# achraf-15/neural_image_compression

Hardware: AMD Instinct MI355X
Metric: images/sec (256x256 RGB, batch 32) fwd+bwd (higher is better)
Workload: dtype f32; 1 GPU; cfg2: JointAutoregressiveHierarchical(M=192,K=1) fwd+rd_loss(lambda=0.01)+bwd+Adam, 32x3x256x256 per GPU, fp32; global_batch=32, parallelism=dp1, step=eager (autograd)

## Files before the change

neural_image_compression_amd/csrc/lic_gdn.hip:

```cpp
#include "lic_common.h"

namespace {

constexpr int GD_BM = 64;
constexpr int GD_BK = 16;

struct GdnParams {
  const float* x;
  const float* g;
  const float* norm;
  const float* w;
  const float* beta;
  const float* res;
  float* out;
  float* out2;
  float* cs_t;
  float* cs_dx;
  long P;
  int inverse;
};

template <int TN, int MODE>
__global__ __launch_bounds__(256) void gdn_kernel(const GdnParams p) {
  static_assert(MODE == 0, "forward only");
  constexpr int C = 64 * TN;
  constexpr int LDX = C + 4;
  constexpr int NCH = C / GD_BK;
  constexpr int SLOTS = GD_BM * C / 4 / 256;
  __shared__ __attribute__((aligned(16))) float smem[GD_BM * LDX];
  const int tid = threadIdx.x, lane = tid & 63;
  const int wave = __builtin_amdgcn_readfirstlane(tid >> 6);
  const int wm0 = (wave >> 1) * 32, wn0 = (wave & 1) * (32 * TN);
  const int li = lane & 31, lh = lane >> 5;
  const long m0 = (long)blockIdx.x * GD_BM;
  const bool inv = p.inverse != 0;

  {
    f32x4 a[SLOTS];
#pragma unroll
    for (int u = 0; u < SLOTS; ++u) {
      const int idx = u * 256 + tid;
      const int row = idx / (C / 4), c4 = (idx - row * (C / 4)) * 4;
      const bool ok = m0 + row < p.P;
      a[u] = *reinterpret_cast<const f32x4*>(p.x + (ok ? (m0 + row) * C + c4 : 0L));
      if (!ok) a[u] = f32x4{0.f, 0.f, 0.f, 0.f};
    }
#pragma unroll
    for (int u = 0; u < SLOTS; ++u) {
      const int idx = u * 256 + tid;
      const int row = idx / (C / 4), c4 = (idx - row * (C / 4)) * 4;
      *reinterpret_cast<f32x4*>(&smem[row * LDX + c4]) = a[u];
    }
  }
  __syncthreads();

  f32x16 acc[TN];
#pragma unroll
  for (int b = 0; b < TN; ++b)
#pragma unroll
    for (int r = 0; r < 16; ++r) acc[b][r] = 0.0f;
  const float* glane = p.w + ((long)(wn0 >> 5) * 512 + lane * 4);
  const float* xrow = smem + (wm0 + li) * LDX + lh * 8;
  f32x4 g0[TN][2], g1[TN][2];
  auto load_g = [&](f32x4 (&rg)[TN][2], int c) {
    const float* src = glane + (long)(c < NCH ? c : NCH - 1) * C * GD_BK;
#pragma unroll
    for (int b = 0; b < TN; ++b) {
      rg[b][0] = *reinterpret_cast<const f32x4*>(src + b * 512);
      rg[b][1] = *reinterpret_cast<const f32x4*>(src + b * 512 + 256);
    }
  };
  auto pool = [&](int c, const f32x4 (&rg)[TN][2]) {
    f32x4 a0 = *reinterpret_cast<const f32x4*>(xrow + c * GD_BK);
    f32x4 a1 = *reinterpret_cast<const f32x4*>(xrow + c * GD_BK + 4);
    a0 = a0 * a0;
    a1 = a1 * a1;
#pragma unroll
    for (int t = 0; t < 8; ++t)
#pragma unroll
      for (int b = 0; b < TN; ++b)
        acc[b] = __builtin_amdgcn_mfma_f32_32x32x2f32((t < 4 ? a0 : a1)[t & 3], rg[b][t >> 2][t & 3], acc[b], 0, 0, 0);
  };
  load_g(g0, 0);
#pragma unroll 1
  for (int c = 0; c < NCH; c += 2) {
    load_g(g1, c + 1);
    pool(c, g0);
    load_g(g0, c + 2);
    pool(c + 1, g1);
  }

  __shared__ __attribute__((aligned(16))) float patch[4][1024];
  float* stg = patch[wave];
  const int c4 = (lane & 7) * 4, r8 = lane >> 3;
  f32x4 csum[TN];
#pragma unroll
  for (int b = 0; b < TN; ++b) csum[b] = f32x4{0.f, 0.f, 0.f, 0.f};
#pragma unroll
  for (int b = 0; b < TN; ++b) {
#pragma unroll
    for (int r = 0; r < 16; ++r) stg[((r & 3) + 8 * (r >> 2) + 4 * lh) * 32 + li] = acc[b][r];
    __builtin_amdgcn_wave_barrier();
    const int col = wn0 + b * 32 + c4;
#pragma unroll
    for (int it = 0; it < 4; ++it) {
      const int rr = it * 8 + r8;
      const long pix = m0 + wm0 + rr;
      if (pix >= p.P) continue;
      const f32x4 s4 = *reinterpret_cast<const f32x4*>(&stg[rr * 32 + c4]);
      const long off = pix * C + col;
      const f32x4 n4 = s4 + *reinterpret_cast<const f32x4*>(p.beta + col);
      const f32x4 x4 = *reinterpret_cast<const f32x4*>(&smem[(wm0 + rr) * LDX + col]);
      f32x4 o;
#pragma unroll
      for (int e = 0; e < 4; ++e)
        o[e] = x4[e] * (inv ? __builtin_amdgcn_sqrtf(n4[e]) : __builtin_amdgcn_rsqf(n4[e]));
      if (p.out2) *reinterpret_cast<f32x4*>(p.out2 + off) = n4;
      if (p.res) o += *reinterpret_cast<const f32x4*>(p.res + off);
      *reinterpret_cast<f32x4*>(p.out + off) = o;
    }
    __builtin_amdgcn_wave_barrier();
  }
}

template <int TN>
__global__ __launch_bounds__(256, 2) void gdn_bwd_reg_kernel(const GdnParams p) {
  constexpr int C = 64 * TN;
  constexpr int LDX = C + 4;
  constexpr int NCH = C / GD_BK;
  __shared__ __attribute__((aligned(16))) float smem[GD_BM * LDX];
  const int tid = threadIdx.x, lane = tid & 63;
  const int wave = __builtin_amdgcn_readfirstlane(tid >> 6);
  const int wm0 = (wave >> 1) * 32, wn0 = (wave & 1) * (32 * TN);
  const int li = lane & 31, lh = lane >> 5;
  const int c4 = (lane & 7) * 4, r8 = lane >> 3;
  const long m0 = (long)blockIdx.x * GD_BM;
  const bool inv = p.inverse != 0;

  f32x4 u[TN][4], xx[TN][4];
#pragma unroll
  for (int b = 0; b < TN; ++b) {
    f32x4 gg[4], nn[4];
    bool ok[4];
#pragma unroll
    for (int it = 0; it < 4; ++it) {
      const long pix = m0 + wm0 + it * 8 + r8;
      ok[it] = pix < p.P;
      const long off = ok[it] ? pix * C + wn0 + b * 32 + c4 : 0L;
      xx[b][it] = *reinterpret_cast<const f32x4*>(p.x + off);
      gg[it] = *reinterpret_cast<const f32x4*>(p.g + off);
      nn[it] = *reinterpret_cast<const f32x4*>(p.norm + off);
    }
#pragma unroll
    for (int it = 0; it < 4; ++it) {
      const int row = wm0 + it * 8 + r8, col = wn0 + b * 32 + c4;
      f32x4 t;
#pragma unroll
      for (int e = 0; e < 4; ++e) {
        const float rs = __builtin_amdgcn_rsqf(nn[it][e]);
        const float gx = gg[it][e] * xx[b][it][e];
        t[e] = inv ? 0.5f * gx * rs : -0.5f * gx * rs * (rs * rs);
        u[b][it][e] = gg[it][e] * (inv ? __builtin_amdgcn_sqrtf(nn[it][e]) : rs);
      }
      if (ok[it]) {
        *reinterpret_cast<f32x4*>(p.out2 + (m0 + row) * C + col) = t;
      } else {
        t = f32x4{0.f, 0.f, 0.f, 0.f};
        u[b][it] = t;
        xx[b][it] = t;
      }
      *reinterpret_cast<f32x4*>(&smem[row * LDX + col]) = t;
    }
  }
  __syncthreads();
  if (p.cs_t && tid < C) {
    float a = 0.0f;
#pragma unroll 8
    for (int r = 0; r < GD_BM; ++r) a += smem[r * LDX + tid];
    p.cs_t[(long)blockIdx.x * C + tid] = a;
  }

  f32x16 acc[TN];
#pragma unroll
  for (int b = 0; b < TN; ++b)
#pragma unroll
    for (int r = 0; r < 16; ++r) acc[b][r] = 0.0f;
  const float* glane = p.w + ((long)(wn0 >> 5) * 512 + lane * 4);
  const float* xrow = smem + (wm0 + li) * LDX + lh * 8;
  f32x4 g0[TN][2], g1[TN][2];
  auto load_g = [&](f32x4 (&rg)[TN][2], int c) {
    const float* src = glane + (long)(c < NCH ? c : NCH - 1) * C * GD_BK;
#pragma unroll
    for (int b = 0; b < TN; ++b) {
      rg[b][0] = *reinterpret_cast<const f32x4*>(src + b * 512);
      rg[b][1] = *reinterpret_cast<const f32x4*>(src + b * 512 + 256);
    }
  };
  auto pool = [&](int c, const f32x4 (&rg)[TN][2]) {
    const f32x4 a0 = *reinterpret_cast<const f32x4*>(xrow + c * GD_BK);
    const f32x4 a1 = *reinterpret_cast<const f32x4*>(xrow + c * GD_BK + 4);
#pragma unroll
    for (int t = 0; t < 8; ++t)
#pragma unroll
      for (int b = 0; b < TN; ++b)
        acc[b] = __builtin_amdgcn_mfma_f32_32x32x2f32((t < 4 ? a0 : a1)[t & 3], rg[b][t >> 2][t & 3], acc[b], 0, 0, 0);
  };
  load_g(g0, 0);
#pragma unroll 1
  for (int c = 0; c < NCH; c += 2) {
    load_g(g1, c + 1);
    pool(c, g0);
    load_g(g0, c + 2);
    pool(c + 1, g1);
  }
  __syncthreads();
  float* stg = smem + wave * 1024;
  f32x4 csum[TN];
#pragma unroll
  for (int b = 0; b < TN; ++b) {
    csum[b] = f32x4{0.f, 0.f, 0.f, 0.f};
#pragma unroll
    for (int r = 0; r < 16; ++r) stg[((r & 3) + 8 * (r >> 2) + 4 * lh) * 32 + li] = acc[b][r];
    __builtin_amdgcn_wave_barrier();
#pragma unroll
    for (int it = 0; it < 4; ++it) {
      const int rr = it * 8 + r8;
      const long pix = m0 + wm0 + rr;
      if (pix >= p.P) continue;
      const f32x4 s4 = *reinterpret_cast<const f32x4*>(&stg[rr * 32 + c4]);
      f32x4 o;
#pragma unroll
      for (int e = 0; e < 4; ++e) o[e] = u[b][it][e] + 2.0f * xx[b][it][e] * s4[e];
      csum[b] += o;
      *reinterpret_cast<f32x4*>(p.out + pix * C + wn0 + b * 32 + c4) = o;
    }
    __builtin_amdgcn_wave_barrier();
  }
  if (p.cs_dx) {
    __syncthreads();
    float* part = smem;
#pragma unroll
    for (int b = 0; b < TN; ++b)
      *reinterpret_cast<f32x4*>(&part[(((wave >> 1) * 8 + r8) * C) + wn0 + b * 32 + c4]) = csum[b];
    __syncthreads();
    if (tid < C) {
      float a = 0.0f;
#pragma unroll
      for (int k = 0; k < 16; ++k) a += part[k * C + tid];
      p.cs_dx[(long)blockIdx.x * C + tid] = a;
    }
  }
}

bool gd_al16(const void* q) { return (reinterpret_cast<uintptr_t>(q) & 15) == 0; }

int gdn_fwd_launch(const GdnParams& p, int C, hipStream_t s) {
  const unsigned grid = (unsigned)cdiv64(p.P, GD_BM);
  if (C == 192)
    hipLaunchKernelGGL((gdn_kernel<3, 0>), dim3(grid), dim3(256), 0, s, p);
  else if (C == 128)
    hipLaunchKernelGGL((gdn_kernel<2, 0>), dim3(grid), dim3(256), 0, s, p);
  else
    hipLaunchKernelGGL((gdn_kernel<1, 0>), dim3(grid), dim3(256), 0, s, p);
  return lic_check_launch();
}

}

LIC_EXPORT int lic_gdn_supported(int32_t C) { return C == 64 || C == 128 || C == 192; }

LIC_EXPORT int lic_gdn_fwd(const float* x, const float* gammaT_packed, const float* beta_eff, const float* res,
                           float* y, float* norm, int64_t P, int32_t C, int32_t inverse, lic_stream_t stream) {
  if (!x || !gammaT_packed || !beta_eff || !y || P <= 0) return LIC_ERR_INVALID;
  if (!lic_gdn_supported(C)) return LIC_ERR_UNSUPPORTED;
  if (!gd_al16(x) || !gd_al16(gammaT_packed) || !gd_al16(beta_eff) || !gd_al16(y) || !gd_al16(norm) || !gd_al16(res))
    return LIC_ERR_INVALID;
  if (P > 0x7FFFFFFFL * 32) return LIC_ERR_UNSUPPORTED;
  GdnParams p{x, nullptr, nullptr, gammaT_packed, beta_eff, res, y, norm, nullptr, nullptr, (long)P, inverse};
  return gdn_fwd_launch(p, C, (hipStream_t)stream);
}

LIC_EXPORT int64_t lic_gdn_bwd_partial_rows(int64_t P) { return P <= 0 ? 0 : cdiv64(P, GD_BM); }

LIC_EXPORT int lic_gdn_bwd(const float* g, const float* x, const float* norm, const float* gamma_packed, float* dx,
                           float* t, float* colsum_t_partial, float* colsum_dx_partial, int64_t P, int32_t C,
                           int32_t inverse, lic_stream_t stream) {
  if (!g || !x || !norm || !gamma_packed || !dx || !t || P <= 0) return LIC_ERR_INVALID;
  if (!lic_gdn_supported(C)) return LIC_ERR_UNSUPPORTED;
  if (!gd_al16(g) || !gd_al16(x) || !gd_al16(norm) || !gd_al16(gamma_packed) || !gd_al16(dx) || !gd_al16(t))
    return LIC_ERR_INVALID;
  if (P > 0x7FFFFFFFL * 32) return LIC_ERR_UNSUPPORTED;
  GdnParams p{x, g, norm, gamma_packed, nullptr, nullptr, dx, t, colsum_t_partial, colsum_dx_partial, (long)P, inverse};
  const unsigned grid = (unsigned)cdiv64(p.P, GD_BM);
  hipStream_t s = (hipStream_t)stream;
  if (C == 192)
    hipLaunchKernelGGL((gdn_bwd_reg_kernel<3>), dim3(grid), dim3(256), 0, s, p);
  else if (C == 128)
    hipLaunchKernelGGL((gdn_bwd_reg_kernel<2>), dim3(grid), dim3(256), 0, s, p);
  else
    hipLaunchKernelGGL((gdn_bwd_reg_kernel<1>), dim3(grid), dim3(256), 0, s, p);
  return lic_check_launch();
}
```

Measured before the change: 1426 images/s.

## Make GDN kernels persistent with two ping-pong wave groups overlapping memory and MFMA

Converts the GDN forward and backward kernels into persistent kernels capped at 256 blocks of 512 threads. Each block holds two 4-wave groups that alternate between a memory phase (load the next tile, finish the previous tile) and an MFMA pooling phase, so global traffic of one group overlaps compute of the other. The goal is to hide memory latency and cut per-block startup cost. In exchange it doubles LDS per block, adds block-wide barriers every half-step, and leaves many compile-time tuning and ablation macros in the code.

```diff
diff --git a/neural_image_compression_amd/csrc/lic_gdn.hip b/neural_image_compression_amd/csrc/lic_gdn.hip
--- a/neural_image_compression_amd/csrc/lic_gdn.hip
+++ b/neural_image_compression_amd/csrc/lic_gdn.hip
@@ -1,9 +1,34 @@
 #include "lic_common.h"
 
+#ifndef GDV_LOADFIRST
+#define GDV_LOADFIRST 1
+#endif
+#ifndef GDV_GPRE
+#define GDV_GPRE 0
+#endif
+#ifndef GDV_PRIO
+#define GDV_PRIO 0
+#endif
+#ifndef GDV_UNROLL
+#define GDV_UNROLL 0
+#endif
+#ifndef GDV_PIN
+#define GDV_PIN 0
+#endif
+#ifndef GDV_LOADFIRST_BWD
+#define GDV_LOADFIRST_BWD GDV_LOADFIRST
+#endif
+#ifndef GDV_PIN_BWD
+#define GDV_PIN_BWD GDV_PIN
+#endif
+#ifndef GDV_ABL
+#define GDV_ABL 0
+#endif
 namespace {
 
 constexpr int GD_BM = 64;
 constexpr int GD_BK = 16;
+constexpr long GD_CUS = 256L;
 
 struct GdnParams {
   const float* x;
@@ -18,50 +43,52 @@
   float* cs_dx;
   long P;
   int inverse;
+  long tiles;
+  int n_iter;
 };
 
+
 template <int TN, int MODE>
-__global__ __launch_bounds__(256) void gdn_kernel(const GdnParams p) {
+__global__ __launch_bounds__(512, 2) void gdn_kernel(const GdnParams p) {
   static_assert(MODE == 0, "forward only");
   constexpr int C = 64 * TN;
   constexpr int LDX = C + 4;
   constexpr int NCH = C / GD_BK;
-  constexpr int SLOTS = GD_BM * C / 4 / 256;
-  __shared__ __attribute__((aligned(16))) float smem[GD_BM * LDX];
-  const int tid = threadIdx.x, lane = tid & 63;
-  const int wave = __builtin_amdgcn_readfirstlane(tid >> 6);
+  constexpr int GROUP = GD_BM * LDX + 4 * 1024;
+  __shared__ __attribute__((aligned(16))) float lds[2 * GROUP];
+  const int lane = threadIdx.x & 63;
+  const int wave8 = __builtin_amdgcn_readfirstlane(threadIdx.x >> 6);
+  const int gi = wave8 >> 2, wave = wave8 & 3;
   const int wm0 = (wave >> 1) * 32, wn0 = (wave & 1) * (32 * TN);
   const int li = lane & 31, lh = lane >> 5;
-  const long m0 = (long)blockIdx.x * GD_BM;
+  const int c4 = (lane & 7) * 4, r8 = lane >> 3;
   const bool inv = p.inverse != 0;
-
-  {
-    f32x4 a[SLOTS];
-#pragma unroll
-    for (int u = 0; u < SLOTS; ++u) {
-      const int idx = u * 256 + tid;
-      const int row = idx / (C / 4), c4 = (idx - row * (C / 4)) * 4;
-      const bool ok = m0 + row < p.P;
-      a[u] = *reinterpret_cast<const f32x4*>(p.x + (ok ? (m0 + row) * C + c4 : 0L));
-      if (!ok) a[u] = f32x4{0.f, 0.f, 0.f, 0.f};
-    }
-#pragma unroll
-    for (int u = 0; u < SLOTS; ++u) {
-      const int idx = u * 256 + tid;
-      const int row = idx / (C / 4), c4 = (idx - row * (C / 4)) * 4;
-      *reinterpret_cast<f32x4*>(&smem[row * LDX + c4]) = a[u];
-    }
-  }
-  __syncthreads();
+  float* smem = lds + gi * GROUP;
+  float* stg = smem + GD_BM * LDX + wave * 1024;
+  auto tile_m0 = [&](int k) { return (2 * ((long)blockIdx.x + (long)k * gridDim.x) + gi) * GD_BM; };
+
+  auto issue = [&](long m0, f32x4 (&a)[TN][4]) {
+#pragma unroll
+    for (int b = 0; b < TN; ++b)
+#pragma unroll
+      for (int it = 0; it < 4; ++it) {
+        const long pix = m0 + wm0 + it * 8 + r8;
+        a[b][it] = f32x4{0.f, 0.f, 0.f, 0.f};
+        if (GDV_ABL == 1 ? pix < -p.P : pix < p.P) a[b][it] = *reinterpret_cast<const f32x4*>(p.x + pix * C + wn0 + b * 32 + c4);
+      }
+  };
+  auto commit = [&](const f32x4 (&a)[TN][4]) {
+#pragma unroll
+    for (int b = 0; b < TN; ++b)
+#pragma unroll
+      for (int it = 0; it < 4; ++it)
+        *reinterpret_cast<f32x4*>(&smem[(wm0 + it * 8 + r8) * LDX + wn0 + b * 32 + c4]) = a[b][it];
+  };
 
   f32x16 acc[TN];
-#pragma unroll
-  for (int b = 0; b < TN; ++b)
-#pragma unroll
-    for (int r = 0; r < 16; ++r) acc[b][r] = 0.0f;
   const float* glane = p.w + ((long)(wn0 >> 5) * 512 + lane * 4);
   const float* xrow = smem + (wm0 + li) * LDX + lh * 8;
-  f32x4 g0[TN][2], g1[TN][2];
+  f32x4 g0[TN][2];
   auto load_g = [&](f32x4 (&rg)[TN][2], int c) {
     const float* src = glane + (long)(c < NCH ? c : NCH - 1) * C * GD_BK;
 #pragma unroll
@@ -70,198 +97,322 @@
       rg[b][1] = *reinterpret_cast<const f32x4*>(src + b * 512 + 256);
     }
   };
-  auto pool = [&](int c, const f32x4 (&rg)[TN][2]) {
-    f32x4 a0 = *reinterpret_cast<const f32x4*>(xrow + c * GD_BK);
-    f32x4 a1 = *reinterpret_cast<const f32x4*>(xrow + c * GD_BK + 4);
-    a0 = a0 * a0;
-    a1 = a1 * a1;
-#pragma unroll
-    for (int t = 0; t < 8; ++t)
+  auto pool_tile = [&]() {
+#pragma unroll
+    for (int b = 0; b < TN; ++b)
+#pragma unroll
+      for (int r = 0; r < 16; ++r) acc[b][r] = 0.0f;
+    if (GDV_ABL == 2) return;
+    if (GDV_PRIO) __builtin_amdgcn_s_setprio(GDV_PRIO);
+    f32x4 g1[TN][2];
+    auto pool = [&](int c, const f32x4 (&rg)[TN][2]) {
+      f32x4 a0 = *reinterpret_cast<const f32x4*>(xrow + c * GD_BK);
+      f32x4 a1 = *reinterpret_cast<const f32x4*>(xrow + c * GD_BK + 4);
+      a0 = a0 * a0;
+      a1 = a1 * a1;
+#pragma unroll
+      for (int t = 0; t < 8; ++t)
+#pragma unroll
+        for (int b = 0; b < TN; ++b)
+          acc[b] = __builtin_amdgcn_mfma_f32_32x32x2f32((t < 4 ? a0 : a1)[t & 3], rg[b][t >> 2][t & 3], acc[b], 0, 0, 0);
+    };
+    if (!GDV_GPRE) load_g(g0, 0);
+#if GDV_UNROLL
+#pragma unroll
+#else
+#pragma unroll 1
+#endif
+    for (int c = 0; c < NCH; c += 2) {
+      load_g(g1, c + 1);
+      pool(c, g0);
+      load_g(g0, c + 2);
+#if GDV_PIN
+      asm volatile("" ::: "memory");
+#endif
+      pool(c + 1, g1);
+    }
+    if (GDV_PRIO) __builtin_amdgcn_s_setprio(0);
+  };
+
+  f32x4 beta4[TN];
+#pragma unroll
+  for (int b = 0; b < TN; ++b) beta4[b] = *reinterpret_cast<const f32x4*>(p.beta + wn0 + b * 32 + c4);
+  auto finish = [&](long m0) {
+    f32x4 r4[TN][4];
+    if (p.res) {
 #pragma unroll
       for (int b = 0; b < TN; ++b)
-        acc[b] = __builtin_amdgcn_mfma_f32_32x32x2f32((t < 4 ? a0 : a1)[t & 3], rg[b][t >> 2][t & 3], acc[b], 0, 0, 0);
-  };
-  load_g(g0, 0);
+#pragma unroll
+        for (int it = 0; it < 4; ++it) {
+          const long pix = m0 + wm0 + it * 8 + r8;
+          if (pix < p.P) r4[b][it] = *reinterpret_cast<const f32x4*>(p.res + pix * C + wn0 + b * 32 + c4);
+        }
+    }
+#pragma unroll
+    for (int b = 0; b < TN; ++b) {
+#pragma unroll
+      for (int r = 0; r < 16; ++r) stg[((r & 3) + 8 * (r >> 2) + 4 * lh) * 32 + li] = acc[b][r];
+      __builtin_amdgcn_wave_barrier();
+      const int col = wn0 + b * 32 + c4;
+#pragma unroll
+      for (int it = 0; it < 4; ++it) {
+        const int rr = it * 8 + r8;
+        const long pix = m0 + wm0 + rr;
+        if (GDV_ABL == 1 ? pix >= -p.P : pix >= p.P) continue;
+        const f32x4 s4 = *reinterpret_cast<const f32x4*>(&stg[rr * 32 + c4]);
+        const long off = pix * C + col;
+        const f32x4 n4 = s4 + beta4[b];
+        const f32x4 x4 = *reinterpret_cast<const f32x4*>(&smem[(wm0 + rr) * LDX + col]);
+        f32x4 o;
+#pragma unroll
+        for (int e = 0; e < 4; ++e)
+          o[e] = x4[e] * (inv ? __builtin_amdgcn_sqrtf(n4[e]) : __builtin_amdgcn_rsqf(n4[e]));
+        if (p.out2) *reinterpret_cast<f32x4*>(p.out2 + off) = n4;
+        if (p.res) o += r4[b][it];
+        *reinterpret_cast<f32x4*>(p.out + off) = o;
+      }
+      __builtin_amdgcn_wave_barrier();
+    }
+  };
+
+  const int last = 2 * p.n_iter;
+  for (int h = 0;; ++h) {
+    const int s = h - gi;
+    if (s >= 0 && s <= last) {
+      const int k = s >> 1;
+      if (s & 1) {
+        pool_tile();
+      } else {
+        f32x4 a[TN][4];
+        if (GDV_LOADFIRST) {
+          if (k < p.n_iter) issue(tile_m0(k), a);
+          if (GDV_GPRE) load_g(g0, 0);
+          if (k > 0) finish(tile_m0(k - 1));
+          if (k < p.n_iter) commit(a);
+        } else {
+          if (k > 0) finish(tile_m0(k - 1));
+          if (GDV_GPRE) load_g(g0, 0);
+          if (k < p.n_iter) {
+            issue(tile_m0(k), a);
+            commit(a);
+          }
+        }
+      }
+    }
+    if (h == last + 1) break;
+    __syncthreads();
+  }
+}
+
+template <int TN>
+__global__ __launch_bounds__(512, 2) void gdn_bwd_reg_kernel(const GdnParams p) {
+  constexpr int C = 64 * TN;
+  constexpr int LDX = C + 4;
+  constexpr int NCH = C / GD_BK;
+  constexpr int GROUP = GD_BM * LDX + 4 * 1024 + 16 * C;
+  __shared__ __attribute__((aligned(16))) float lds[2 * GROUP];
+  const int tid = threadIdx.x & 255, lane = tid & 63;
+  const int wave8 = __builtin_amdgcn_readfirstlane(threadIdx.x >> 6);
+  const int gi = wave8 >> 2, wave = wave8 & 3;
+  const int wm0 = (wave >> 1) * 32, wn0 = (wave & 1) * (32 * TN);
+  const int li = lane & 31, lh = lane >> 5;
+  const int c4 = (lane & 7) * 4, r8 = lane >> 3;
+  const bool inv = p.inverse != 0;
+  float* smem = lds + gi * GROUP;
+  float* stg = smem + GD_BM * LDX + wave * 1024;
+  float* part = smem + GD_BM * LDX + 4 * 1024;
+  auto tile_of = [&](int k) { return 2 * ((long)blockIdx.x + (long)k * gridDim.x) + gi; };
+
+  f32x4 u[TN][4], xx[TN][4];
+  auto issue_b = [&](long m0, int b, f32x4 (&nx)[4], f32x4 (&ng)[4], f32x4 (&nn)[4]) {
+#pragma unroll
+    for (int it = 0; it < 4; ++it) {
+      const long pix = m0 + wm0 + it * 8 + r8;
+      nx[it] = f32x4{0.f, 0.f, 0.f, 0.f};
+      ng[it] = f32x4{0.f, 0.f, 0.f, 0.f};
+      nn[it] = f32x4{1.f, 1.f, 1.f, 1.f};
+      if (GDV_ABL == 1 ? pix < -p.P : pix < p.P) {
+        const long off = pix * C + wn0 + b * 32 + c4;
+        nx[it] = *reinterpret_cast<const f32x4*>(p.x + off);
+        ng[it] = *reinterpret_cast<const f32x4*>(p.g + off);
+        nn[it] = *reinterpret_cast<const f32x4*>(p.norm + off);
+      }
+    }
+  };
+  auto convert_b = [&](long m0, int b, const f32x4 (&nx)[4], const f32x4 (&ng)[4], const f32x4 (&nn)[4]) {
+#pragma unroll
+    for (int it = 0; it < 4; ++it) {
+      const int row = wm0 + it * 8 + r8, col = wn0 + b * 32 + c4;
+      const bool ok = m0 + row < p.P;
+      f32x4 t;
+#pragma unroll
+      for (int e = 0; e < 4; ++e) {
+        const float rs = __builtin_amdgcn_rsqf(nn[it][e]);
+        const float gx = ng[it][e] * nx[it][e];
+        t[e] = inv ? 0.5f * gx * rs : -0.5f * gx * rs * (rs * rs);
+        u[b][it][e] = ng[it][e] * (inv ? __builtin_amdgcn_sqrtf(nn[it][e]) : rs);
+      }
+      xx[b][it] = nx[it];
+      if (GDV_ABL == 1 ? m0 + row < -p.P : ok) {
+        *reinterpret_cast<f32x4*>(p.out2 + (m0 + row) * C + col) = t;
+      } else if (!ok) {
+        t = f32x4{0.f, 0.f, 0.f, 0.f};
+        u[b][it] = t;
+        xx[b][it] = t;
+      }
+      *reinterpret_cast<f32x4*>(&smem[row * LDX + col]) = t;
+    }
+  };
+
+  auto fold_t = [&](long tile) {
+    if (tile < p.tiles && tid < C) {
+      float a = 0.0f;
+#pragma unroll 8
+      for (int r = 0; r < GD_BM; ++r) a += smem[r * LDX + tid];
+      p.cs_t[tile * C + tid] = a;
+    }
+  };
+
+  f32x16 acc[TN];
+  const float* glane = p.w + ((long)(wn0 >> 5) * 512 + lane * 4);
+  const float* xrow = smem + (wm0 + li) * LDX + lh * 8;
+  f32x4 g0[TN][2];
+  auto load_g = [&](f32x4 (&rg)[TN][2], int c) {
+    const float* src = glane + (long)(c < NCH ? c : NCH - 1) * C * GD_BK;
+#pragma unroll
+    for (int b = 0; b < TN; ++b) {
+      rg[b][0] = *reinterpret_cast<const f32x4*>(src + b * 512);
+      rg[b][1] = *reinterpret_cast<const f32x4*>(src + b * 512 + 256);
+    }
+  };
+  auto pool_tile = [&]() {
+#pragma unroll
+    for (int b = 0; b < TN; ++b)
+#pragma unroll
+      for (int r = 0; r < 16; ++r) acc[b][r] = 0.0f;
+    if (GDV_ABL == 2) return;
+    if (GDV_PRIO) __builtin_amdgcn_s_setprio(GDV_PRIO);
+    f32x4 g1[TN][2];
+    auto pool = [&](int c, const f32x4 (&rg)[TN][2]) {
+      const f32x4 a0 = *reinterpret_cast<const f32x4*>(xrow + c * GD_BK);
+      const f32x4 a1 = *reinterpret_cast<const f32x4*>(xrow + c * GD_BK + 4);
+#pragma unroll
+      for (int t = 0; t < 8; ++t)
+#pragma unroll
+        for (int b = 0; b < TN; ++b)
+          acc[b] = __builtin_amdgcn_mfma_f32_32x32x2f32((t < 4 ? a0 : a1)[t & 3], rg[b][t >> 2][t & 3], acc[b], 0, 0, 0);
+    };
+    if (!GDV_GPRE) load_g(g0, 0);
+#if GDV_UNROLL
+#pragma unroll
+#else
 #pragma unroll 1
-  for (int c = 0; c < NCH; c += 2) {
-    load_g(g1, c + 1);
-    pool(c, g0);
-    load_g(g0, c + 2);
-    pool(c + 1, g1);
-  }
-
-  __shared__ __attribute__((aligned(16))) float patch[4][1024];
-  float* stg = patch[wave];
-  const int c4 = (lane & 7) * 4, r8 = lane >> 3;
-  f32x4 csum[TN];
-#pragma unroll
-  for (int b = 0; b < TN; ++b) csum[b] = f32x4{0.f, 0.f, 0.f, 0.f};
-#pragma unroll
-  for (int b = 0; b < TN; ++b) {
+#endif
+    for (int c = 0; c < NCH; c += 2) {
+      load_g(g1, c + 1);
+      pool(c, g0);
+      load_g(g0, c + 2);
+#if GDV_PIN_BWD
+      asm volatile("" ::: "memory");
+#endif
+      pool(c + 1, g1);
+    }
+    if (GDV_PRIO) __builtin_amdgcn_s_setprio(0);
+  };
+
+  auto finish_b = [&](long m0, int b) {
+    f32x4 csum = f32x4{0.f, 0.f, 0.f, 0.f};
 #pragma unroll
     for (int r = 0; r < 16; ++r) stg[((r & 3) + 8 * (r >> 2) + 4 * lh) * 32 + li] = acc[b][r];
     __builtin_amdgcn_wave_barrier();
-    const int col = wn0 + b * 32 + c4;
 #pragma unroll
     for (int it = 0; it < 4; ++it) {
       const int rr = it * 8 + r8;
       const long pix = m0 + wm0 + rr;
-      if (pix >= p.P) continue;
-      const f32x4 s4 = *reinterpret_cast<const f32x4*>(&stg[rr * 32 + c4]);
-      const long off = pix * C + col;
-      const f32x4 n4 = s4 + *reinterpret_cast<const f32x4*>(p.beta + col);
-      const f32x4 x4 = *reinterpret_cast<const f32x4*>(&smem[(wm0 + rr) * LDX + col]);
-      f32x4 o;
-#pragma unroll
-      for (int e = 0; e < 4; ++e)
-        o[e] = x4[e] * (inv ? __builtin_amdgcn_sqrtf(n4[e]) : __builtin_amdgcn_rsqf(n4[e]));
-      if (p.out2) *reinterpret_cast<f32x4*>(p.out2 + off) = n4;
-      if (p.res) o += *reinterpret_cast<const f32x4*>(p.res + off);
-      *reinterpret_cast<f32x4*>(p.out + off) = o;
-    }
-    __builtin_amdgcn_wave_barrier();
-  }
-}
-
-template <int TN>
-__global__ __launch_bounds__(256, 2) void gdn_bwd_reg_kernel(const GdnParams p) {
-  constexpr int C = 64 * TN;
-  constexpr int LDX = C + 4;
-  constexpr int NCH = C / GD_BK;
-  __shared__ __attribute__((aligned(16))) float smem[GD_BM * LDX];
-  const int tid = threadIdx.x, lane = tid & 63;
-  const int wave = __builtin_amdgcn_readfirstlane(tid >> 6);
-  const int wm0 = (wave >> 1) * 32, wn0 = (wave & 1) * (32 * TN);
-  const int li = lane & 31, lh = lane >> 5;
-  const int c4 = (lane & 7) * 4, r8 = lane >> 3;
-  const long m0 = (long)blockIdx.x * GD_BM;
-  const bool inv = p.inverse != 0;
-
-  f32x4 u[TN][4], xx[TN][4];
-#pragma unroll
-  for (int b = 0; b < TN; ++b) {
-    f32x4 gg[4], nn[4];
-    bool ok[4];
-#pragma unroll
-    for (int it = 0; it < 4; ++it) {
-      const long pix = m0 + wm0 + it * 8 + r8;
-      ok[it] = pix < p.P;
-      const long off = ok[it] ? pix * C + wn0 + b * 32 + c4 : 0L;
-      xx[b][it] = *reinterpret_cast<const f32x4*>(p.x + off);
-      gg[it] = *reinterpret_cast<const f32x4*>(p.g + off);
-      nn[it] = *reinterpret_cast<const f32x4*>(p.norm + off);
-    }
-#pragma unroll
-    for (int it = 0; it < 4; ++it) {
-      const int row = wm0 + it * 8 + r8, col = wn0 + b * 32 + c4;
-      f32x4 t;
-#pragma unroll
-      for (int e = 0; e < 4; ++e) {
-        const float rs = __builtin_amdgcn_rsqf(nn[it][e]);
-        const float gx = gg[it][e] * xx[b][it][e];
-        t[e] = inv ? 0.5f * gx * rs : -0.5f * gx * rs * (rs * rs);
-        u[b][it][e] = gg[it][e] * (inv ? __builtin_amdgcn_sqrtf(nn[it][e]) : rs);
-      }
-      if (ok[it]) {
-        *reinterpret_cast<f32x4*>(p.out2 + (m0 + row) * C + col) = t;
-      } else {
-        t = f32x4{0.f, 0.f, 0.f, 0.f};
-        u[b][it] = t;
-        xx[b][it] = t;
-      }
-      *reinterpret_cast<f32x4*>(&smem[row * LDX + col]) = t;
-    }
-  }
-  __syncthreads();
-  if (p.cs_t && tid < C) {
-    float a = 0.0f;
-#pragma unroll 8
-    for (int r = 0; r < GD_BM; ++r) a += smem[r * LDX + tid];
-    p.cs_t[(long)blockIdx.x * C + tid] = a;
-  }
-
-  f32x16 acc[TN];
-#pragma unroll
-  for (int b = 0; b < TN; ++b)
-#pragma unroll
-    for (int r = 0; r < 16; ++r) acc[b][r] = 0.0f;
-  const float* glane = p.w + ((long)(wn0 >> 5) * 512 + lane * 4);
-  const float* xrow = smem + (wm0 + li) * LDX + lh * 8;
-  f32x4 g0[TN][2], g1[TN][2];
-  auto load_g = [&](f32x4 (&rg)[TN][2], int c) {
-    const float* src = glane + (long)(c < NCH ? c : NCH - 1) * C * GD_BK;
-#pragma unroll
-    for (int b = 0; b < TN; ++b) {
-      rg[b][0] = *reinterpret_cast<const f32x4*>(src + b * 512);
-      rg[b][1] = *reinterpret_cast<const f32x4*>(src + b * 512 + 256);
-    }
-  };
-  auto pool = [&](int c, const f32x4 (&rg)[TN][2]) {
-    const f32x4 a0 = *reinterpret_cast<const f32x4*>(xrow + c * GD_BK);
-    const f32x4 a1 = *reinterpret_cast<const f32x4*>(xrow + c * GD_BK + 4);
-#pragma unroll
-    for (int t = 0; t < 8; ++t)
-#pragma unroll
-      for (int b = 0; b < TN; ++b)
-        acc[b] = __builtin_amdgcn_mfma_f32_32x32x2f32((t < 4 ? a0 : a1)[t & 3], rg[b][t >> 2][t & 3], acc[b], 0, 0, 0);
-  };
-  load_g(g0, 0);
-#pragma unroll 1
-  for (int c = 0; c < NCH; c += 2) {
-    load_g(g1, c + 1);
-    pool(c, g0);
-    load_g(g0, c + 2);
-    pool(c + 1, g1);
-  }
-  __syncthreads();
-  float* stg = smem + wave * 1024;
-  f32x4 csum[TN];
-#pragma unroll
-  for (int b = 0; b < TN; ++b) {
-    csum[b] = f32x4{0.f, 0.f, 0.f, 0.f};
-#pragma unroll
-    for (int r = 0; r < 16; ++r) stg[((r & 3) + 8 * (r >> 2) + 4 * lh) * 32 + li] = acc[b][r];
-    __builtin_amdgcn_wave_barrier();
-#pragma unroll
-    for (int it = 0; it < 4; ++it) {
-      const int rr = it * 8 + r8;
-      const long pix = m0 + wm0 + rr;
-      if (pix >= p.P) continue;
+      if (GDV_ABL == 1 ? pix >= -p.P : pix >= p.P) continue;
       const f32x4 s4 = *reinterpret_cast<const f32x4*>(&stg[rr * 32 + c4]);
       f32x4 o;
 #pragma unroll
       for (int e = 0; e < 4; ++e) o[e] = u[b][it][e] + 2.0f * xx[b][it][e] * s4[e];
-      csum[b] += o;
+      csum += o;
       *reinterpret_cast<f32x4*>(p.out + pix * C + wn0 + b * 32 + c4) = o;
     }
     __builtin_amdgcn_wave_barrier();
+    if (p.cs_dx) *reinterpret_cast<f32x4*>(&part[(((wave >> 1) * 8 + r8) * C) + wn0 + b * 32 + c4]) = csum;
+  };
+  auto memory_step = [&](bool fin, long m_fin, bool ld, long m_ld) {
+    if (GDV_LOADFIRST_BWD) {
+#pragma unroll
+      for (int b = 0; b < TN; ++b) {
+        f32x4 nx[4], ng[4], nn[4];
+        if (ld) issue_b(m_ld, b, nx, ng, nn);
+        if (GDV_GPRE && b == 0) load_g(g0, 0);
+        if (fin) finish_b(m_fin, b);
+        if (ld) convert_b(m_ld, b, nx, ng, nn);
+      }
+    } else {
+#pragma unroll
+      for (int b = 0; b < TN; ++b)
+        if (fin) finish_b(m_fin, b);
+      if (GDV_GPRE) load_g(g0, 0);
+      if (ld) {
+#pragma unroll
+        for (int b = 0; b < TN; ++b) {
+          f32x4 nx[4], ng[4], nn[4];
+          issue_b(m_ld, b, nx, ng, nn);
+          convert_b(m_ld, b, nx, ng, nn);
+        }
+      }
+    }
+  };
+
+  auto fold_dx = [&](long tile) {
+    if (tile < p.tiles && tid < C) {
+      float a = 0.0f;
+#pragma unroll
+      for (int k = 0; k < 16; ++k) a += part[k * C + tid];
+      p.cs_dx[tile * C + tid] = a;
+    }
+  };
+
+  const int last = 2 * p.n_iter + 1;
+  for (int h = 0;; ++h) {
+    const int s = h - gi;
+    if (s >= 0 && s <= last) {
+      const int k = s >> 1;
+      if (s & 1) {
+        if (k > 0 && p.cs_dx) fold_dx(tile_of(k - 1));
+        if (k < p.n_iter) {
+          if (p.cs_t) fold_t(tile_of(k));
+          pool_tile();
+        }
+      } else {
+        memory_step(k > 0, tile_of(k - 1) * GD_BM, k < p.n_iter, tile_of(k) * GD_BM);
+      }
+    }
+    if (h == last + 1) break;
+    __syncthreads();
   }
-  if (p.cs_dx) {
-    __syncthreads();
-    float* part = smem;
-#pragma unroll
-    for (int b = 0; b < TN; ++b)
-      *reinterpret_cast<f32x4*>(&part[(((wave >> 1) * 8 + r8) * C) + wn0 + b * 32 + c4]) = csum[b];
-    __syncthreads();
-    if (tid < C) {
-      float a = 0.0f;
-#pragma unroll
-      for (int k = 0; k < 16; ++k) a += part[k * C + tid];
-      p.cs_dx[(long)blockIdx.x * C + tid] = a;
-    }
-  }
 }
 
 bool gd_al16(const void* q) { return (reinterpret_cast<uintptr_t>(q) & 15) == 0; }
 
-int gdn_fwd_launch(const GdnParams& p, int C, hipStream_t s) {
-  const unsigned grid = (unsigned)cdiv64(p.P, GD_BM);
+unsigned gdn_plan(GdnParams& p) {
+  p.tiles = cdiv64(p.P, GD_BM);
+  const long pairs = (p.tiles + 1) / 2;
+  const long grid = pairs < GD_CUS ? pairs : GD_CUS;
+  p.n_iter = (int)((p.tiles + 2 * grid - 1) / (2 * grid));
+  return (unsigned)grid;
+}
+
+int gdn_fwd_launch(GdnParams& p, int C, hipStream_t s) {
+  const unsigned grid = gdn_plan(p);
   if (C == 192)
-    hipLaunchKernelGGL((gdn_kernel<3, 0>), dim3(grid), dim3(256), 0, s, p);
+    hipLaunchKernelGGL((gdn_kernel<3, 0>), dim3(grid), dim3(512), 0, s, p);
   else if (C == 128)
-    hipLaunchKernelGGL((gdn_kernel<2, 0>), dim3(grid), dim3(256), 0, s, p);
+    hipLaunchKernelGGL((gdn_kernel<2, 0>), dim3(grid), dim3(512), 0, s, p);
   else
-    hipLaunchKernelGGL((gdn_kernel<1, 0>), dim3(grid), dim3(256), 0, s, p);
+    hipLaunchKernelGGL((gdn_kernel<1, 0>), dim3(grid), dim3(512), 0, s, p);
   return lic_check_launch();
 }
 
@@ -276,7 +427,7 @@
   if (!gd_al16(x) || !gd_al16(gammaT_packed) || !gd_al16(beta_eff) || !gd_al16(y) || !gd_al16(norm) || !gd_al16(res))
     return LIC_ERR_INVALID;
   if (P > 0x7FFFFFFFL * 32) return LIC_ERR_UNSUPPORTED;
-  GdnParams p{x, nullptr, nullptr, gammaT_packed, beta_eff, res, y, norm, nullptr, nullptr, (long)P, inverse};
+  GdnParams p{x, nullptr, nullptr, gammaT_packed, beta_eff, res, y, norm, nullptr, nullptr, (long)P, inverse, 0, 0};
   return gdn_fwd_launch(p, C, (hipStream_t)stream);
 }
 
@@ -290,14 +441,14 @@
   if (!gd_al16(g) || !gd_al16(x) || !gd_al16(norm) || !gd_al16(gamma_packed) || !gd_al16(dx) || !gd_al16(t))
     return LIC_ERR_INVALID;
   if (P > 0x7FFFFFFFL * 32) return LIC_ERR_UNSUPPORTED;
-  GdnParams p{x, g, norm, gamma_packed, nullptr, nullptr, dx, t, colsum_t_partial, colsum_dx_partial, (long)P, inverse};
-  const unsigned grid = (unsigned)cdiv64(p.P, GD_BM);
+  GdnParams p{x, g, norm, gamma_packed, nullptr, nullptr, dx, t, colsum_t_partial, colsum_dx_partial, (long)P, inverse, 0, 0};
+  const unsigned grid = gdn_plan(p);
   hipStream_t s = (hipStream_t)stream;
   if (C == 192)
-    hipLaunchKernelGGL((gdn_bwd_reg_kernel<3>), dim3(grid), dim3(256), 0, s, p);
+    hipLaunchKernelGGL((gdn_bwd_reg_kernel<3>), dim3(grid), dim3(512), 0, s, p);
   else if (C == 128)
-    hipLaunchKernelGGL((gdn_bwd_reg_kernel<2>), dim3(grid), dim3(256), 0, s, p);
+    hipLaunchKernelGGL((gdn_bwd_reg_kernel<2>), dim3(grid), dim3(512), 0, s, p);
   else
-    hipLaunchKernelGGL((gdn_bwd_reg_kernel<1>), dim3(grid), dim3(256), 0, s, p);
+    hipLaunchKernelGGL((gdn_bwd_reg_kernel<1>), dim3(grid), dim3(512), 0, s, p);
   return lic_check_launch();
 }
```

Measured after the change: 1402 images/s. 1.7% lower.
